# linum-uqam/ViT-OCM-WMSegmentation

Measured on AMD Instinct MI355X. Metric: OCM tiles/s (224x224, ViT-S/16 attention-map inference), higher is better.
Workload: dtype bf16x3

## Files before the change

include/ocm_vit.h:

```cpp
#ifndef OCM_VIT_H
#define OCM_VIT_H

#include <stddef.h>
#include <stdint.h>

#ifdef __cplusplus
extern "C" {
#endif

#define OCM_ABI_VERSION 16

enum {
    OCM_OK = 0,
    OCM_EINVAL = 1,
    OCM_ESTATE = 2,
    OCM_EHIP = 3,
    OCM_ENOMEM = 4,
    OCM_ENAME = 5
};

enum {
    OCM_PREC_BF16 = 0,
    OCM_PREC_FP32 = 1,
    OCM_PREC_BF16X3 = 2
// ... 82 lines not shown

int ocm_op_cast_bf16(const float *src, void *dst_bf16, size_t count, void *stream);
int ocm_op_cast_split(const float *src, void *dst_split, size_t count, void *stream);
int ocm_op_merge_split(const void *src_split, float *dst, size_t count, void *stream);

enum {
    OCM_EPI_BIAS_F32 = 0,
    OCM_EPI_BIAS_RESID_F32 = 1,
    OCM_EPI_BIAS_GELU_BF16 = 2,
    OCM_EPI_BIAS_BF16 = 3
};

int ocm_op_linear(int32_t precision, const void *a, const void *w, const float *bias, const float *resid,
                  void *out, int32_t M, int32_t N, int32_t K, int32_t epilogue, void *stream);

int ocm_linear_resid_ln_supported(int32_t D);
int ocm_op_linear_resid_ln(int32_t precision, const void *a, const void *w, const float *bias, const float *resid,
                           float *x, const float *gamma, const float *beta, void *xn, int32_t M, int32_t D, int32_t K,
                           float eps, void *stream);

int32_t ocm_n_pad(int32_t n_tokens);
int32_t ocm_n_pad_prec(int32_t precision, int32_t n_tokens);

int ocm_op_qkv_proj(int32_t precision, const void *a, const void *w, const float *bias, void *q, void *k,
                    void *vt, float *qkv_f32, int32_t batch, int32_t n_tokens, int32_t heads,
                    void *stream);

int ocm_op_attention(int32_t precision, const void *q, const void *k, const void *vt, void *ctx, float *lse2,
                     int32_t batch, int32_t n_tokens, int32_t heads, float scale, void *stream);

// ... 154 lines not shown
```

vit-ocm-wmsegmentation_amd/_lib.py:

```python
import ctypes as C
import os

_HERE = os.path.dirname(os.path.abspath(__file__))
LIB_PATH = os.environ.get("OCM_VIT_LIB") or os.path.join(_HERE, "libocm_vit.so")

OCM_ABI_VERSION = 16
OCM_OK, OCM_EINVAL, OCM_ESTATE, OCM_EHIP, OCM_ENOMEM, OCM_ENAME = 0, 1, 2, 3, 4, 5

OCM_PREC_BF16 = 0
OCM_PREC_FP32 = 1
OCM_PREC_BF16X3 = 2
OCM_SWIN_OPT_FUSE_MLP = 0
PRECISIONS = {"bf16": OCM_PREC_BF16, "fp32": OCM_PREC_FP32, "bf16x3": OCM_PREC_BF16X3}
DEFAULT_PRECISION = "bf16x3"
OCM_LN_F32, OCM_LN_BF16, OCM_LN_SPLIT = 0, 1, 2
OCM_OPT_FUSE_LN = 0
OCM_OPT_FOLD_LN = 1

OCM_OUT_FEAT = 1 << 0
OCM_OUT_ATTN = 1 << 1
OCM_OUT_QKV = 1 << 2
OCM_OUT_TOKENS = 1 << 3
OCM_OUT_ROWS = 1 << 4
OCM_LAST_ATTN_ONLY = 1 << 5
# ... 79 lines not shown
    "ocm_vit_destroy": (None, [_vp]),
    "ocm_vit_set_param": (C.c_int, [_vp, C.c_char_p, _vp, _sz, _vp]),
    "ocm_vit_params_ready": (C.c_int, [_vp]),
    "ocm_vit_workspace_bytes": (_sz, [_vp, _i32, _i32]),
    "ocm_vit_forward": (C.c_int, [_vp, C.POINTER(OcmVitIO)]),
    "ocm_vit_prepare_tokens": (C.c_int, [_vp, C.POINTER(OcmVitIO), _vp]),
    "ocm_vit_block_forward": (C.c_int, [_vp, _i32, _vp, _i32, _i32, _i32, _vp, _vp, _vp, _sz, _vp]),
    "ocm_vit_final_norm": (C.c_int, [_vp, _vp, _vp, _i64, _vp]),
    "ocm_op_layernorm": (C.c_int, [_vp, _vp, _vp, _vp, _i32, _i64, _i32, _f32, _vp]),
    "ocm_op_cast_bf16": (C.c_int, [_vp, _vp, _sz, _vp]),
    "ocm_op_cast_split": (C.c_int, [_vp, _vp, _sz, _vp]),
    "ocm_op_merge_split": (C.c_int, [_vp, _vp, _sz, _vp]),
    "ocm_n_pad_prec": (_i32, [_i32, _i32]),
    "ocm_op_linear": (C.c_int, [_i32, _vp, _vp, _vp, _vp, _vp, _i32, _i32, _i32, _i32, _vp]),
    "ocm_linear_resid_ln_supported": (C.c_int, [_i32]),
    "ocm_op_linear_resid_ln": (C.c_int, [_i32, _vp, _vp, _vp, _vp, _vp, _vp, _vp, _vp, _i32, _i32, _i32, _f32, _vp]),
    "ocm_n_pad": (_i32, [_i32]),
    "ocm_op_qkv_proj": (C.c_int, [_i32, _vp, _vp, _vp, _vp, _vp, _vp, _vp, _i32, _i32, _i32, _vp]),
    "ocm_op_attention": (C.c_int, [_i32, _vp, _vp, _vp, _vp, _vp, _i32, _i32, _i32, _f32, _vp]),
    "ocm_op_qkv_proj_hd": (C.c_int, [_i32, _vp, _vp, _vp, _vp, _vp, _vp, _vp, _i32, _i32, _i32, _i32, _vp]),
    "ocm_op_attention_hd": (C.c_int, [_i32, _vp, _vp, _vp, _vp, _vp, _i32, _i32, _i32, _i32, _f32, _vp]),
    "ocm_op_attention_probs_hd": (C.c_int, [_i32, _vp, _vp, _vp, _vp, _i32, _i32, _i32, _i32, _f32, _vp]),
    "ocm_op_attention_generic": (C.c_int, [C.c_int32, C.c_void_p, C.c_void_p, C.c_void_p, C.c_int32, C.c_int32, C.c_int32,
                                           C.c_int32, C.c_float, C.c_void_p]),
    "ocm_op_attention_probs": (C.c_int, [_i32, _vp, _vp, _vp, _vp, _i32, _i32, _i32, _f32, _vp]),
    "ocm_op_attention_rows": (C.c_int, [_i32, _vp, _vp, _vp, _i32, _vp, _i32, _i32, _i32, _f32, _vp]),
    "ocm_op_attention_map": (C.c_int, [_vp, _vp, _i32, _i32, _i32, _i32, _i32, _i32, _i32, _vp]),
    "ocm_op_tile_postprocess": (C.c_int, [_vp, _vp, _i32, _i32, _i32, _i32, _vp]),
    "ocm_op_bilinear_upsample": (C.c_int, [_vp, _vp, _i32, _i32, _i32, _i32, _vp]),
    "ocm_op_nearest_upsample": (C.c_int, [_vp, _vp, _i32, _i32, _i32, _i32, _vp]),
# ... 130 lines not shown
```

vit-ocm-wmsegmentation_amd/csrc/common.h:

```cpp
#pragma once
#include <hip/hip_runtime.h>
#include <stddef.h>
#include <stdint.h>

typedef __bf16 bf16;
typedef __bf16 bf16x2 __attribute__((ext_vector_type(2)));
typedef __bf16 bf16x4 __attribute__((ext_vector_type(4)));
typedef __bf16 bf16x8 __attribute__((ext_vector_type(8)));
typedef float f32x2 __attribute__((ext_vector_type(2)));
typedef float f32x4 __attribute__((ext_vector_type(4)));
typedef float f32x16 __attribute__((ext_vector_type(16)));

#define OCM_WAVE 64
#define OCM_HEAD_DIM 64

__device__ __forceinline__ int acc_row32(int reg, int h) { return (reg & 3) + 8 * (reg >> 2) + 4 * h; }

__device__ __forceinline__ int lds_off(int row, int chunk) {
    return row * 128 + ((chunk ^ ((row >> 1) & 7)) << 4);
}

__device__ __forceinline__ void lds_barrier() {
    __builtin_amdgcn_fence(__ATOMIC_RELEASE, "workgroup", "local");
    __builtin_amdgcn_s_barrier();
// ... 54 lines not shown
#if defined(OCM_ABL) && OCM_ABL == 1
    asm volatile("" ::"v"(ah), "v"(al), "v"(bh), "v"(bl));
    return c;
#endif
    c = __builtin_amdgcn_mfma_f32_32x32x16_bf16(al, bh, c, 0, 0, 0);
    c = __builtin_amdgcn_mfma_f32_32x32x16_bf16(ah, bl, c, 0, 0, 0);
    return __builtin_amdgcn_mfma_f32_32x32x16_bf16(ah, bh, c, 0, 0, 0);
}

typedef float f32x4_t __attribute__((ext_vector_type(4)));
__device__ __forceinline__ f32x4_t mfma16x3(bf16x8 ah, bf16x8 al, bf16x8 bh, bf16x8 bl, f32x4_t c) {
    c = __builtin_amdgcn_mfma_f32_16x16x32_bf16(al, bh, c, 0, 0, 0);
    c = __builtin_amdgcn_mfma_f32_16x16x32_bf16(ah, bl, c, 0, 0, 0);
    return __builtin_amdgcn_mfma_f32_16x16x32_bf16(ah, bh, c, 0, 0, 0);
}
__device__ __forceinline__ bf16x8 tr_read8(const char *p) {
#if defined(__HIP_DEVICE_COMPILE__)
    typedef short s16x4 __attribute__((ext_vector_type(4)));
    typedef __attribute__((address_space(3))) s16x4 *lds_s16x4;
    const s16x4 a = __builtin_amdgcn_ds_read_tr16_b64_v4i16((lds_s16x4)p);
    const s16x4 b = __builtin_amdgcn_ds_read_tr16_b64_v4i16((lds_s16x4)(p + 4 * 64));
    typedef short s16x8 __attribute__((ext_vector_type(8)));
    const s16x8 v = {a[0], a[1], a[2], a[3], b[0], b[1], b[2], b[3]};
    return __builtin_bit_cast(bf16x8, v);
#else
    return bf16x8{};
#endif
}

template <int ACCL>
__device__ __forceinline__ int acc_rpos(int e, int lane) {
    return ACCL ? 16 * (e >> 3) + 4 * ((lane >> 4) & 3) + (e & 3) : acc_row32(e, lane >> 5);
}
template <int ACCL>
__device__ __forceinline__ int acc_cpos(int e, int lane) {
    return ACCL ? 16 * ((e >> 2) & 1) + (lane & 15) : (lane & 31);
}

__device__ __forceinline__ int xcd_remap(int bid, int nwg) {
    const int q = nwg >> 3, r = nwg & 7, x = bid & 7;
    return (x < r ? x * (q + 1) : r * (q + 1) + (x - r) * q) + (bid >> 3);
}

__device__ __forceinline__ void xcd_remap2(int &bx, int &by) {
    const int id = xcd_remap(blockIdx.y * gridDim.x + blockIdx.x, gridDim.x * gridDim.y);
    by = id / (int)gridDim.x;
    bx = id - by * (int)gridDim.x;
}

__device__ __forceinline__ float fast_exp2(float x) { return __builtin_amdgcn_exp2f(x); }

// ... 37 lines not shown
```

vit-ocm-wmsegmentation_amd/csrc/engine.hip:

```cpp
#include <stdarg.h>
#include <stdio.h>
#include <string.h>

#include <atomic>
#include <mutex>
#include <string>
#include <vector>

#include "host_common.h"
#include "launch.h"
#include "dev_knobs.h"

static thread_local std::string g_err;

int ocm_fail(int code, const char *fmt, ...) {
    char buf[512];
    va_list ap;
    va_start(ap, fmt);
    vsnprintf(buf, sizeof buf, fmt, ap);
    va_end(ap);
    g_err = buf;
    return code;
}
#define fail ocm_fail
// ... 673 lines not shown
                             void *out, int32_t M, int32_t N, int32_t K, int32_t epilogue, void *stream) {
    int pc = 0, rc = prec_of(precision, &pc);
    if (rc) return rc;
    if (!a || !w || !out) return fail(OCM_EINVAL, "null argument");
    const int kq = pc ? 32 : 64;
    if (M <= 0 || N <= 0 || N % 32 || K <= 0 || K % kq)
        return fail(OCM_EINVAL, "bad shape M=%d N=%d K=%d (N%%32, K%%%d)", M, N, K, kq);
    if (pc == 2 && (epilogue == OCM_EPI_BIAS_GELU_BF16 || epilogue == OCM_EPI_BIAS_BF16) && N % 32)
        return fail(OCM_EINVAL, "split-pair outputs need N %% 32 == 0");
    if (epilogue < 0 || epilogue > 3) return fail(OCM_EINVAL, "bad epilogue %d", epilogue);
    if (epilogue == OCM_EPI_BIAS_RESID_F32 && !resid) return fail(OCM_EINVAL, "residual epilogue without resid");
    HIP_TRY(launch_linear(pc, a, w, bias, resid, out, M, N, K, epilogue, (hipStream_t)stream));
    return OCM_OK;
}

extern "C" int ocm_linear_resid_ln_supported(int32_t D) { return linear_resid_ln_supported(D) ? 1 : 0; }

extern "C" int ocm_op_linear_resid_ln(int32_t precision, const void *a, const void *w, const float *bias,
                                      const float *resid, float *x, const float *gamma, const float *beta, void *xn,
                                      int32_t M, int32_t D, int32_t K, float eps, void *stream) {
    int pc = 0, rc = prec_of(precision, &pc);
    if (rc) return rc;
    if (!a || !w || !resid || !x || !gamma || !beta || !xn) return fail(OCM_EINVAL, "null argument");
    if (!linear_resid_ln_supported(D)) return fail(OCM_EINVAL, "row width %d not in {128, 256, 384}", D);
    if (M <= 0 || K <= 0 || K % 64) return fail(OCM_EINVAL, "bad shape M=%d K=%d (K%%64)", M, K);
    HIP_TRY(launch_linear_resid_ln(pc, a, w, bias, resid, x, gamma, beta, xn, M, D, K, eps, (hipStream_t)stream));
    return OCM_OK;
}

static int op_qkv_proj(int32_t precision, const void *a, const void *w, const float *bias, void *q, void *k, void *vt,
// ... 303 lines not shown
```

vit-ocm-wmsegmentation_amd/csrc/gemm_core.h:

```cpp
#pragma once
#include <type_traits>
#include "common.h"

#ifdef OCM_GEMM_STAMPS
__device__ unsigned long long g_wstamps[512 * 16 * 8];
#define WSTAMP(k)                                                                                       \
    do {                                                                                                \
        if (t == nsteps / 2 && (threadIdx.x & 63) == 0 && blockIdx.x < 512)                              \
            g_wstamps[(blockIdx.x * 16 + (threadIdx.x >> 6 & 15)) * 8 + (k)] = __builtin_readcyclecounter(); \
    } while (0)
__device__ unsigned long long g_stamps[8192 * 8];
#define STAMP(i)                                                                                        \
    do {                                                                                                \
        if (threadIdx.x == 0 && blockIdx.x < 8192) g_stamps[blockIdx.x * 8 + (i)] = __builtin_readcyclecounter(); \
    } while (0)
#else
#define STAMP(i) ((void)0)
#define WSTAMP(k) ((void)0)
#endif

template <int BM_, int BN_, int WAVES_M_, int WAVES_N_, int MF16_ = 0>
struct GemmCfg {
    static constexpr int BM = BM_, BN = BN_, WAVES_M = WAVES_M_, WAVES_N = WAVES_N_, MF16 = MF16_;
    static constexpr int NT = WAVES_M * WAVES_N * OCM_WAVE;
// ... 53 lines not shown
#endif
        return *(const Raw *)(h + t * 128 + c * 16);
    }
    __device__ __forceinline__ static Raw finish(const Raw &r, int) { return r; }
};

template <class AL, class = void>
struct aload_w_tail {
    static constexpr bool v = false;
};
template <class AL>
struct aload_w_tail<AL, std::void_t<decltype(AL::W_TAIL)>> {
    static constexpr bool v = AL::W_TAIL;
};

template <class Cfg, class E, bool SWAP>
__device__ __forceinline__ void mma_step(const char *Ab, const char *Bb, int r, int h,
                                         f32x16 (&acc)[Cfg::TM][Cfg::TN], int wm = 0) {
    constexpr int TM = Cfg::TM, TN = Cfg::TN;
    static_assert(!Cfg::HALF || (Elem<E>::MODE == 2 && Cfg::MF16 && !SWAP), "half tiles exist on the 16 x 16 shape only");
    if constexpr (Elem<E>::MODE == 2 && Cfg::MF16) {
        const int r16 = r & 15, g = (r >> 4) + 2 * h;
        bf16x8 ah[TM][2], al[TM][2], bh[TN][2], bl[TN][2];
#pragma unroll
        for (int i = 0; i < TM; ++i)
#pragma unroll
            for (int ra = 0; ra < 2; ++ra) {
                if (Cfg::HALF && i == TM - 1) {
                    if (ra == 0) {
                        const char *Ah = Ab + ((TM - 1) * Cfg::RB - wm * 16) * 128;
                        ah[i][0] = *(const bf16x8 *)(Ah + lds_off(r16, g));
                        al[i][0] = *(const bf16x8 *)(Ah + lds_off(r16, 4 + g));
                    }
                    continue;
                }
                ah[i][ra] = *(const bf16x8 *)(Ab + i * Cfg::RB * 128 + lds_off(ra * 16 + r16, g));
                al[i][ra] = *(const bf16x8 *)(Ab + i * Cfg::RB * 128 + lds_off(ra * 16 + r16, 4 + g));
            }
#pragma unroll
        for (int j = 0; j < TN; ++j)
#pragma unroll
            for (int cb = 0; cb < 2; ++cb) {
                bh[j][cb] = *(const bf16x8 *)(Bb + j * Cfg::CB * 128 + lds_off(cb * 16 + r16, g));
                bl[j][cb] = *(const bf16x8 *)(Bb + j * Cfg::CB * 128 + lds_off(cb * 16 + r16, 4 + g));
            }
#pragma unroll
        for (int i = 0; i < TM; ++i)
#pragma unroll
            for (int j = 0; j < TN; ++j)
#pragma unroll
                for (int q = 0; q < ((Cfg::HALF && i == TM - 1) ? 2 : 4); ++q) {
                    f32x4_t c = __builtin_shufflevector(acc[i][j], acc[i][j], 0, 1, 2, 3);
                    if (q == 1) c = __builtin_shufflevector(acc[i][j], acc[i][j], 4, 5, 6, 7);
                    if (q == 2) c = __builtin_shufflevector(acc[i][j], acc[i][j], 8, 9, 10, 11);
                    if (q == 3) c = __builtin_shufflevector(acc[i][j], acc[i][j], 12, 13, 14, 15);
                    c = SWAP ? mfma16x3(bh[j][q >> 1], bl[j][q >> 1], ah[i][q & 1], al[i][q & 1], c)
                             : mfma16x3(ah[i][q >> 1], al[i][q >> 1], bh[j][q & 1], bl[j][q & 1], c);
#pragma unroll
                    for (int e = 0; e < 4; ++e) acc[i][j][4 * q + e] = c[e];
                }
    } else if constexpr (Elem<E>::MODE == 2) {
#pragma unroll
        for (int s = 0; s < 2; ++s) {
            bf16x8 ah[TM], al[TM], bh[TN], bl[TN];
#pragma unroll
            for (int i = 0; i < TM; ++i) {
                ah[i] = *(const bf16x8 *)(Ab + i * Cfg::RB * 128 + lds_off(r, 2 * s + h));
                al[i] = *(const bf16x8 *)(Ab + i * Cfg::RB * 128 + lds_off(r, 4 + 2 * s + h));
            }
#pragma unroll
            for (int j = 0; j < TN; ++j) {
// ... 234 lines not shown
        __builtin_amdgcn_raw_ptr_buffer_load_lds(rs, (lds_ptr)(img + (j * NW + wave) * 1024), 16, voff[j], soff, 0, AUX);
#endif
}

template <int CNT, int AUX = 0>
__device__ __forceinline__ void dma_pieces(__amdgpu_buffer_rsrc_t rs, char *img, const int (&voff)[CNT], const int (&piece)[CNT],
                                           int soff) {
#if defined(__HIP_DEVICE_COMPILE__)
    typedef __attribute__((address_space(3))) void *lds_ptr;
#pragma unroll
    for (int j = 0; j < CNT; ++j)
        __builtin_amdgcn_raw_ptr_buffer_load_lds(rs, (lds_ptr)(img + piece[j] * 1024), 16, voff[j], soff, 0, AUX);
#endif
}

template <class Cfg, class E, bool SWAP, int KSTEPS, int NSTAGE, int A_AUX = 0>
__device__ __forceinline__ void gemm_mainloop_dma(const E *__restrict__ A, int64_t lda, const E *__restrict__ W,
                                                  int64_t ldw, int m0, int n0, int M, int N, int K, char *smem,
                                                  f32x16 (&acc)[Cfg::TM][Cfg::TN], const float *__restrict__ bias) {
    constexpr int BM = Cfg::BM, BN = Cfg::BN, NT = Cfg::NT, NW = NT / 64;
    constexpr int TM = Cfg::TM, TN = Cfg::TN;
    constexpr int A_P = BM / 8, A_I = (A_P + NW - 1) / NW, B_I = BN / 8 / NW, LPS = A_I + B_I;
    constexpr int STAGE = (BM + BN) * 128, D = NSTAGE - 1;
    static_assert(BM % 8 == 0 && BN % (8 * NW) == 0 && (A_P % NW == 0 || 2 * (A_P % NW) >= NW), "each wave fills whole groups of 8 rows");
    static_assert(NSTAGE >= 2 && NSTAGE <= 4, "2..4 LDS stages");
    const int tid = threadIdx.x, lane = tid & 63;
    const int wave = __builtin_amdgcn_readfirstlane(tid >> 6);
    const int wm = wave / Cfg::WAVES_N, wn = wave % Cfg::WAVES_N;
    const int r = lane & 31, h = lane >> 5;
    const int esz = (int)sizeof(E);
    const int nsteps = KSTEPS > 0 ? KSTEPS : K / Elem<E>::KROW;

    auto bound = [](int64_t rows, int64_t ld_bytes) {
        const int64_t b = rows * ld_bytes;
// ... 4 lines not shown
    const auto rsB = __builtin_amdgcn_make_buffer_rsrc((void *)((const char *)W + (int64_t)n0 * ldw * esz), 0,
                                                       bound(N - n0, ldw * esz), 0x00020000);
    int voffA[A_I], voffB[B_I];
    int pieceA[A_I];
#pragma unroll
    for (int j = 0; j < A_I; ++j) {
        int pc = j * NW + wave;
        if (pc >= A_P) pc -= A_P % NW;
        pieceA[j] = pc;
        const int rho = pc * 8 + (lane >> 3);
        voffA[j] = rho * (int)(lda * esz) + (((lane & 7) ^ ((rho >> 1) & 7)) << 4);
    }
#pragma unroll
    for (int j = 0; j < B_I; ++j) {
        const int rho = (j * NW + wave) * 8 + (lane >> 3);
        voffB[j] = rho * (int)(ldw * esz) + (((lane & 7) ^ ((rho >> 1) & 7)) << 4);
    }
#define OCM_DMA_ISSUE(t, buf)                                                   \
    do {                                                                        \
        char *st_ = smem + (buf) * STAGE;                                       \
        dma_pieces<A_I, A_AUX>(rsA, st_, voffA, pieceA, (t) * 128);             \
        dma_rows<B_I, NW>(rsB, st_ + BM * 128, voffB, wave, (t) * 128);         \
    } while (0)
    auto compute = [&](int buf) {
        const char *st = smem + buf * STAGE;
        mma_step<Cfg, E, SWAP>(st + (wm * 32) * 128, st + BM * 128 + (wn * 32) * 128, r, h, acc, wm);
    };

    constexpr int ACCL = accl_of<Cfg, E>();
    constexpr int NBV = SWAP ? 16 : (ACCL ? 2 : 1);
    float bv[TN][NBV];
#pragma unroll
    for (int j = 0; j < TN; ++j) {
        const int nb = n0 + (j * Cfg::WAVES_N + wn) * 32;
#pragma unroll
        for (int e = 0; e < NBV; ++e)
            bv[j][e] = bias ? bias[min(nb + (SWAP ? acc_rpos<ACCL>(e, lane) : acc_cpos<ACCL>(4 * e, lane)), N - 1)] : 0.f;
    }
#pragma unroll
    for (int t = 0; t < D; ++t)
        if (t < nsteps) OCM_DMA_ISSUE(t, t);
#pragma unroll
    for (int j = 0; j < TN; ++j)
#pragma unroll
        for (int i = 0; i < TM; ++i)
#pragma unroll
            for (int e = 0; e < 16; ++e) acc[i][j][e] = bv[j][SWAP ? e : (ACCL ? ((e >> 2) & 1) : 0)];
    int bc = 0, bi = D % NSTAGE;
#ifdef OCM_GEMM_STAMPS
    unsigned long long stamp_wait = 0;
#endif
    for (int t = 0; t < nsteps; ++t) {
        const int younger = min(D - 1, nsteps - 1 - t);
#ifdef OCM_GEMM_STAMPS
        const unsigned long long tw0 = __builtin_readcyclecounter();
#endif
        WSTAMP(0);
        wait_vm_steps<LPS, NSTAGE - 2>(younger);
        WSTAMP(1);
#ifdef OCM_GEMM_STAMPS
        const unsigned long long tw1 = __builtin_readcyclecounter();
#endif
        raw_barrier();
#ifdef OCM_GEMM_STAMPS
        if (t == 0) STAMP(6);
        if (t > 0) {
            const unsigned long long tw2 = __builtin_readcyclecounter();
            stamp_wait += ((tw2 - tw1) << 32) | ((tw1 - tw0) & 0xFFFFFFFFull);
        }
#endif
        WSTAMP(2);
#if !defined(OCM_ABL) || OCM_ABL != 2
        if (t + D < nsteps) OCM_DMA_ISSUE(t + D, bi);
#endif
        __builtin_amdgcn_sched_barrier(0);
        WSTAMP(3);
        compute(bc);
#ifdef OCM_GEMM_STAMPS
        if (t == nsteps / 2) {
            __builtin_amdgcn_sched_barrier(0);
            asm volatile("v_mov_b32 %0, %0\n\ts_nop 0" : "+v"(acc[TM - 1][TN - 1][15]));
            WSTAMP(4);
        }
#endif
        bc = bc + 1 == NSTAGE ? 0 : bc + 1;
        bi = bi + 1 == NSTAGE ? 0 : bi + 1;
    }
    raw_barrier();
#ifdef OCM_GEMM_STAMPS
    if (threadIdx.x == 0 && blockIdx.x < 8192) g_stamps[blockIdx.x * 8 + 7] = stamp_wait;
#endif
#undef OCM_DMA_ISSUE
}

constexpr int EPI_MAXS = 6;
struct EpiPre {
    f32x2 raw[EPI_MAXS];
    f32x2 cd;
};
struct EpiNoPre {};
template <class Cfg, class Epi>
__device__ __forceinline__ auto epi_prefetch(const Epi &epi, int m0, int n0, int M, int N) {
    if constexpr (Epi::ROWTAB) {
// ... 71 lines not shown
        constexpr int NBUF = 2 * PASS <= LDS_AVAIL ? 2 : 1;
#pragma unroll
        for (int j = 0; j < Cfg::TN; ++j) {
            if (NBUF == 1 && j) lds_barrier();
            float *C = (float *)(smem + (j % NBUF) * PASS);
            if (active)
#pragma unroll
            for (int i = 0; i < Cfg::TM; ++i) {
                const int col0 = (i * Cfg::WAVES_M + wm) * 32;
#pragma unroll
                for (int e = 0; e < 16; ++e)
                    C[(wn * 32 + acc_rpos<ACCL>(e, lane)) * Cfg::BM + col0 + acc_cpos<ACCL>(e, lane)] = acc[i][j][e];
            }
            lds_barrier();
            if (active) epi.template run<PassCfg<Cfg::BM, Cfg::CB, Cfg::NT>>((const float *)C, m0, n0 + j * Cfg::CB, rowtab, coltab + j * Cfg::CB);
        }
    }
}

template <class Cfg, class E, bool SWAP, int KSTEPS, int NSTAGE, class Epi, int A_AUX = 0>
__global__ __launch_bounds__(Cfg::NT) void gemm_dma_kernel(const E *__restrict__ A, int64_t lda, const E *__restrict__ W,
                                                           int64_t ldw, int M, int N, int K, Epi epi) {
    extern __shared__ __attribute__((aligned(16))) char smem[];
    const int tiles_n = (N + Cfg::BN - 1) / Cfg::BN;
    const int id = xcd_remap(blockIdx.x, gridDim.x);
    const int tm = id / tiles_n, tn = id - tm * tiles_n;
    const int m0 = tm * Cfg::BM, n0 = tn * Cfg::BN;
    f32x16 acc[Cfg::TM][Cfg::TN];
    const auto pre = epi_prefetch<Cfg>(epi, m0, n0, M, N);
    STAMP(0);
#if defined(OCM_ABL) && OCM_ABL == 4
#pragma unroll
    for (int i = 0; i < Cfg::TM; ++i)
#pragma unroll
        for (int j = 0; j < Cfg::TN; ++j)
#pragma unroll
            for (int e = 0; e < 16; ++e) acc[i][j][e] = (float)(threadIdx.x + e);
#else
    gemm_mainloop_dma<Cfg, E, SWAP, KSTEPS, NSTAGE, A_AUX>(A, lda, W, ldw, m0, n0, M, N, K, smem, acc, epi.bias);
#endif
    STAMP(1);
#if defined(OCM_ABL) && OCM_ABL == 3
#pragma unroll
    for (int i = 0; i < Cfg::TM; ++i)
#pragma unroll
        for (int j = 0; j < Cfg::TN; ++j) asm volatile("" ::"v"(acc[i][j]));
#else
    run_epilogue<Cfg, SWAP, Epi, NSTAGE * (Cfg::BM + Cfg::BN) * 128, decltype(pre), accl_of<Cfg, E>()>(acc, smem, epi, m0, n0, true, &pre);
#endif
    STAMP(4);
#ifdef OCM_GEMM_STAMPS
    __builtin_amdgcn_s_waitcnt(0);
    STAMP(5);
// ... 24 lines not shown
```

vit-ocm-wmsegmentation_amd/csrc/gemm_kernels.h:

```cpp
#pragma once
#include <type_traits>
#include "gemm_core.h"
#include "launch.h"
#include "dev_knobs.h"

int ocm_wt_mask();

#ifndef OCM_SMALLM_STAGES
#define OCM_SMALLM_STAGES 4
#endif
constexpr int OCM_SMALLM_ROWS = 4096;
typedef GemmCfg<128, 128, 2, 2> Cfg128x128;
typedef GemmCfg<128, 128, 2, 4> Cfg128x128q;
typedef GemmCfg<128, 128, 2, 4, 1> Cfg128x128q16;
typedef GemmCfg<128, 128, 2, 2, 1> Cfg128x128m16;
typedef GemmCfg<160, 128, 2, 4, 1> Cfg160x128q16;
typedef GemmCfg<256, 256, 2, 4, 1> Cfg256x256m16;
typedef GemmCfg<64, 128, 2, 2> Cfg64x128;
typedef GemmCfg<64, 128, 2, 4> Cfg64x128w;
typedef GemmCfg<64, 64, 2, 2> Cfg64x64;
typedef GemmCfg<256, 256, 2, 4> Cfg256x256;

static inline bool big_tiles_pay(int M, int N, int K) {
    return K >= 768 && N % 256 == 0 && (long)((M + 255) / 256) * (N / 256) >= 512;
// ... 61 lines not shown
}
__device__ __forceinline__ f32x2 ln_col_entry(const LnFold &ln, int n) {
    return ln.stats ? f32x2{ln.c[n], ln.d[n]} : f32x2{0.f, 0.f};
}

template <int MODE, class OE>
struct EpiLinear {
    const float *bias;
    const float *resid;
    void *out;
    int M, N;
    int64_t ldo;
    int wt = 0;
    LnFold ln;
    static constexpr bool ROWTAB = (MODE == 2 || MODE == 3);
    __device__ __forceinline__ void row_raw(int m, f32x2 (&raw)[EPI_MAXS]) const { ln_row_raw(ln, m, raw); }
    __device__ __forceinline__ f32x2 row_final(const f32x2 (&raw)[EPI_MAXS]) const { return ln_row_final(ln, raw); }
    __device__ __forceinline__ f32x2 col_entry(int n) const { return ln_col_entry(ln, n); }
    template <class Cfg>
    __device__ __forceinline__ void run(const float *C, int m0, int n0, const f32x2 *rowtab, const f32x2 *coltab) const {
        constexpr int BM = Cfg::BM, BN = Cfg::BN, NT = Cfg::NT;
        constexpr bool ACT_OUT = (MODE == 2 || MODE == 3);
        constexpr int W = ACT_OUT ? Elem<OE>::EPW : 4;
        constexpr int CPR = BN / W;
        constexpr int TOTAL = BM * CPR, ITERS = (TOTAL + NT - 1) / NT;
        f32x4 rs[MODE == 1 ? ITERS : 1];
        if (MODE == 1) {
#pragma unroll
            for (int i = 0; i < ITERS; ++i) {
                const int q = min((int)threadIdx.x + i * NT, TOTAL - 1), row = q / CPR, col = (q - row * CPR) * W;
// ... 21 lines not shown
                    const f32x2 mr = rowtab[row];
                    const float mu = mr[0], rstd = mr[1];
#pragma unroll
                    for (int e = 0; e < 4; ++e) {
                        const f32x2 cd = coltab[col + e];
                        v0[e] = fmaf(rstd, fmaf(-mu, cd[0], v0[e]), cd[1]);
                    }
                    if (W == 8) {
#pragma unroll
                        for (int e = 0; e < 4; ++e) {
                            const f32x2 cd = coltab[col + 4 + e];
                            v1[e] = fmaf(rstd, fmaf(-mu, cd[0], v1[e]), cd[1]);
                        }
                    }
                }
                if (MODE == 2) {
#pragma unroll
                    for (int e = 0; e < 4; e += 2) {
                        const f32x2 a = gelu_erf2(f32x2{v0[e], v0[e + 1]});
                        v0[e] = a[0];
                        v0[e + 1] = a[1];
                        if (W == 8) {
                            const f32x2 b = gelu_erf2(f32x2{v1[e], v1[e + 1]});
                            v1[e] = b[0];
                            v1[e + 1] = b[1];
                        }
                    }
                }
                if (wt)
                    store_act_wt((OE *)nullptr, (char *)out + (int64_t)m * ldo * (int)sizeof(OE), n, v0, v1);
                else
                    store_act((OE *)nullptr, (char *)out + (int64_t)m * ldo * (int)sizeof(OE), n, v0, v1);
            }
        }
    }
};

template <class OE>
struct EpiResidStats {
    static constexpr bool ROWTAB = false;
    static constexpr int BN_MULT = 64;
    const float *bias;
    const float *resid;
    float *x;
    void *xs;
    float *stats;
    int M, N;
// ... 157 lines not shown
typedef GemmCfg<128, 192, 4, 2> Cfg128x192;
typedef GemmCfg<128, 256, 2, 4> Cfg128x256;
typedef GemmCfg<128, 96, 4, 1> Cfg128x96;
template <class Epi, class = void>
struct epi_bn_mult {
    static constexpr int v = 1;
};
template <class Epi>
struct epi_bn_mult<Epi, std::void_t<decltype(Epi::BN_MULT)>> {
    static constexpr int v = Epi::BN_MULT;
};

template <int MODE, class E, class Epi>
static hipError_t launch_linear_epi(const E *a, const E *w, const Epi &epi, int M, int N, int K, hipStream_t s) {
    RowLoader<E> al{a, K};
    if constexpr (Elem<E>::MODE == 2) {
#ifdef OCM_DEV
        switch (OCM_KNOB(0)) {
            case -1: goto reg_staged;
            case 1: if (N % 256 == 0) return launch_gemm_dma<Cfg256x256, E, 2>(a, K, w, K, M, N, K, epi, s); break;
            case 4: if (N % 128 == 0) return launch_gemm_dma<Cfg128x128, E, 2>(a, K, w, K, M, N, K, epi, s); break;
            case 6: if (N % 128 == 0) return launch_gemm_dma<Cfg256x128, E, 2>(a, K, w, K, M, N, K, epi, s); break;
            case 7: if (N % 128 == 0) return launch_gemm_dma<Cfg64x128, E, 2>(a, K, w, K, M, N, K, epi, s); break;
            case 8: if (N % 128 == 0) return launch_gemm_dma<Cfg64x128, E, 3>(a, K, w, K, M, N, K, epi, s); break;
            case 9: if (N % 128 == 0) return launch_gemm_dma<Cfg64x128, E, 4>(a, K, w, K, M, N, K, epi, s); break;
            case 10: if (N % 64 == 0) return launch_gemm_dma<Cfg64x64, E, 4>(a, K, w, K, M, N, K, epi, s); break;
            case 11: if (N == 384) return launch_gemm_dma<Cfg128x192, E, 3>(a, K, w, K, M, N, K, epi, s); break;
            case 12: if (N % 128 == 0) return launch_gemm_dma<Cfg128x128q, E, 2>(a, K, w, K, M, N, K, epi, s); break;
            case 13: if (N % 128 == 0) return launch_gemm_dma<Cfg128x128q16, E, 2>(a, K, w, K, M, N, K, epi, s); break;
            case 14: if (N % 128 == 0) return launch_gemm_dma<Cfg128x128m16, E, 2>(a, K, w, K, M, N, K, epi, s); break;
// ... 716 lines not shown
```

vit-ocm-wmsegmentation_amd/csrc/kernels_gemm.hip:

```cpp
#include "launch.h"
#include "dev_knobs.h"

template <class E>
hipError_t launch_linear_e(const E *a, const E *w, const float *bias, const float *resid, void *out, int M, int N, int K,
                           int epilogue, hipStream_t s, const LnFold &ln, const StatsOut &so);
template <class E>
hipError_t launch_linear_ld_e(const E *a, int64_t lda, const E *w, const float *bias, const float *resid, void *out,
                              int64_t ldo, int M, int N, int K, int epilogue, hipStream_t s);
template <class E>
hipError_t launch_resid_ln_e(const E *a, const E *w, const float *bias, const float *resid, float *x, const float *gamma,
                             const float *beta, void *xn, int M, int D, int K, float eps, hipStream_t s);
template <class E>
hipError_t launch_qkv_e(const E *a, const E *w, const float *bias, E *q, E *k, E *vt, float *qkv_f32, int batch,
                        int n_tokens, int n_pad, int heads, int head_dim, bool want_v, hipStream_t s, const LnFold &ln);
template <class E>
hipError_t launch_patch_e(const PatchArgs &pa, const E *w, const float *bias, const float *pos, float *x, int dim,
                          hipStream_t s, const StatsOut &so);

#ifdef OCM_DEV
int g_ocm_knobs[8] = {0, 0, 0, 0, 0, 0, 0, 0};
#endif
int ocm_wt_mask() { return OCM_KNOB(1) == 0 ? 35 : OCM_KNOB(1) < 0 ? 0 : OCM_KNOB(1); }

hipError_t launch_linear_ld(int prec, const void *a, int64_t lda, const void *w, const float *bias, const float *resid,
                            void *out, int64_t ldo, int M, int N, int K, int epilogue, hipStream_t s) {
    if (prec == 2) return hipErrorInvalidValue;
    if (prec)
        return launch_linear_ld_e<float>((const float *)a, lda, (const float *)w, bias, resid, out, ldo, M, N, K, epilogue,
                                         s);
    return launch_linear_ld_e<bf16>((const bf16 *)a, lda, (const bf16 *)w, bias, resid, out, ldo, M, N, K, epilogue, s);
}

hipError_t launch_linear(int prec, const void *a, const void *w, const float *bias, const float *resid, void *out, int M,
                         int N, int K, int epilogue, hipStream_t s, const LnFold &ln, const StatsOut &so) {
    if (prec == 2) return launch_linear_e<sp32>((const sp32 *)a, (const sp32 *)w, bias, resid, out, M, N, K, epilogue, s, ln, so);
    if (prec) return launch_linear_e<float>((const float *)a, (const float *)w, bias, resid, out, M, N, K, epilogue, s, ln, so);
    return launch_linear_e<bf16>((const bf16 *)a, (const bf16 *)w, bias, resid, out, M, N, K, epilogue, s, ln, so);
// ... 35 lines not shown
```

vit-ocm-wmsegmentation_amd/csrc/launch.h:

```cpp
#pragma once
#include <atomic>
#include "common.h"

typedef std::atomic<unsigned long long> OptinMask;
static inline hipError_t lds_optin(const void *kern, int bytes, OptinMask &done) {
    int dev = 0;
    if (hipError_t e = hipGetDevice(&dev); e != hipSuccess) return e;
    const unsigned long long bit = 1ull << (dev & 63);
    if (done.load(std::memory_order_acquire) & bit) return hipSuccess;
    const hipError_t e = hipFuncSetAttribute(kern, hipFuncAttributeMaxDynamicSharedMemorySize, bytes);
    if (e == hipSuccess) done.fetch_or(bit, std::memory_order_release);
    return e;
}

hipError_t launch_layernorm(const float *x, const float *gamma, const float *beta, void *y, int out_kind,
                            int64_t rows, int dim, float eps, hipStream_t s);
static inline int ln_kind_of_prec(int prec) { return prec == 0 ? 1 : prec == 1 ? 0 : 2; }
hipError_t launch_cast_bf16(const float *src, bf16 *dst, size_t count, hipStream_t s);
hipError_t launch_cast_split(const float *src, void *dst, size_t count, hipStream_t s);
hipError_t launch_merge_split(const void *src, float *dst, size_t count, hipStream_t s);
hipError_t launch_fold_split(const float *src, void *dst, int D, int C, int pp, hipStream_t s);
hipError_t launch_fold_cast_bf16(const float *src, bf16 *dst, int D, int C, int pp, hipStream_t s);
hipError_t launch_fold_f32(const float *src, float *dst, int D, int C, int pp, hipStream_t s);
hipError_t launch_im2col3x3(int prec, const float *in, void *out, int batch, int h, int w, int C, int relu, hipStream_t s);
// ... 15 lines not shown
    const float *tok_shift = nullptr;
    float *part = nullptr;
};
constexpr int OCM_SPLITK = 4, OCM_SPLITK_MAX_ROWS = 512;
hipError_t launch_splitk_finish(const float *part, int slices, const float *bias, const float *resid, float *x, void *xs,
                                float *stats, int M, int N, hipStream_t s, const StatsOut &so = StatsOut());
hipError_t launch_cls_rows_stats(const float *cls, const float *pos, float *x, void *xs, float *stats, int batch,
                                 int n_tokens, int dim, hipStream_t s, float *shift = nullptr, float *tok_shift = nullptr,
                                 const float *pe_bias = nullptr);
hipError_t launch_fold_ln(const float *W, const float *gamma, const float *beta, const float *bias, void *Wf, float *cvec,
                          float *dvec, int N, int K, hipStream_t s);

hipError_t launch_linear(int prec, const void *a, const void *w, const float *bias, const float *resid, void *out, int M,
                         int N, int K, int epilogue, hipStream_t s, const LnFold &ln = LnFold(),
                         const StatsOut &so = StatsOut());
bool linear_resid_ln_supported(int D);
hipError_t launch_linear_resid_ln(int prec, const void *a, const void *w, const float *bias, const float *resid, float *x,
                                  const float *gamma, const float *beta, void *xn, int M, int D, int K, float eps,
                                  hipStream_t s);
hipError_t launch_qkv(int prec, const void *a, const void *w, const float *bias, void *q, void *k, void *vt,
                      float *qkv_f32, int batch, int n_tokens, int n_pad, int heads, int head_dim, bool want_v,
                      hipStream_t s, const LnFold &ln = LnFold());
hipError_t launch_attention_generic(int prec, const float *qkv, void *ctx, float *attn, const int32_t *query_rows,
                                    int n_rows, float *rows, int batch, int n_tokens, int heads, int head_dim, float scale,
                                    hipStream_t s);
struct PatchArgs {
    const float *image;
    int64_t sb, sc, sy;
    const int32_t *origins;
    int batch, hp, wp, p, chans;
// ... 80 lines not shown
```

Baseline: 28970.

## Store bf16 GEMM epilogue directly from registers using a transposed MFMA order

For split-bf16 GEMMs with bias or bias+GELU bf16 epilogues on 128-wide N tiles, the mainloop now runs in swapped operand order with a permuted W row mapping. Each lane then holds eight contiguous output columns, so the epilogue stores straight from accumulators instead of staging the tile through LDS. The LN-fold row and column tables are published to LDS just before the last k-step, and the final barrier is dropped. A forced-tile test entry point is also added. This risks bank conflicts or correctness issues from the new row permutation.

```diff
diff --git a/include/ocm_vit.h b/include/ocm_vit.h
--- a/include/ocm_vit.h
+++ b/include/ocm_vit.h
@@ -120,6 +120,9 @@
 int ocm_op_linear(int32_t precision, const void *a, const void *w, const float *bias, const float *resid,
                   void *out, int32_t M, int32_t N, int32_t K, int32_t epilogue, void *stream);
 
+int ocm_op_linear_tile(int32_t precision, const void *a, const void *w, const float *bias, void *out, int32_t M, int32_t N,
+                       int32_t K, int32_t epilogue, int32_t tile_rows, void *stream);
+
 int ocm_linear_resid_ln_supported(int32_t D);
 int ocm_op_linear_resid_ln(int32_t precision, const void *a, const void *w, const float *bias, const float *resid,
                            float *x, const float *gamma, const float *beta, void *xn, int32_t M, int32_t D, int32_t K,
diff --git a/vit-ocm-wmsegmentation_amd/_lib.py b/vit-ocm-wmsegmentation_amd/_lib.py
--- a/vit-ocm-wmsegmentation_amd/_lib.py
+++ b/vit-ocm-wmsegmentation_amd/_lib.py
@@ -117,6 +117,7 @@
     "ocm_n_pad_prec": (_i32, [_i32, _i32]),
     "ocm_op_linear": (C.c_int, [_i32, _vp, _vp, _vp, _vp, _vp, _i32, _i32, _i32, _i32, _vp]),
     "ocm_linear_resid_ln_supported": (C.c_int, [_i32]),
+    "ocm_op_linear_tile": (C.c_int, [_i32, _vp, _vp, _vp, _vp, _i32, _i32, _i32, _i32, _i32, _vp]),
     "ocm_op_linear_resid_ln": (C.c_int, [_i32, _vp, _vp, _vp, _vp, _vp, _vp, _vp, _vp, _i32, _i32, _i32, _f32, _vp]),
     "ocm_n_pad": (_i32, [_i32]),
     "ocm_op_qkv_proj": (C.c_int, [_i32, _vp, _vp, _vp, _vp, _vp, _vp, _vp, _i32, _i32, _i32, _vp]),
diff --git a/vit-ocm-wmsegmentation_amd/csrc/common.h b/vit-ocm-wmsegmentation_amd/csrc/common.h
--- a/vit-ocm-wmsegmentation_amd/csrc/common.h
+++ b/vit-ocm-wmsegmentation_amd/csrc/common.h
@@ -92,6 +92,11 @@
     c = __builtin_amdgcn_mfma_f32_16x16x32_bf16(ah, bl, c, 0, 0, 0);
     return __builtin_amdgcn_mfma_f32_16x16x32_bf16(ah, bh, c, 0, 0, 0);
 }
+__device__ __forceinline__ f32x4_t mfma16x3_t(bf16x8 ah, bf16x8 al, bf16x8 bh, bf16x8 bl, f32x4_t c) {
+    c = __builtin_amdgcn_mfma_f32_16x16x32_bf16(bh, al, c, 0, 0, 0);
+    c = __builtin_amdgcn_mfma_f32_16x16x32_bf16(bl, ah, c, 0, 0, 0);
+    return __builtin_amdgcn_mfma_f32_16x16x32_bf16(bh, ah, c, 0, 0, 0);
+}
 __device__ __forceinline__ bf16x8 tr_read8(const char *p) {
 #if defined(__HIP_DEVICE_COMPILE__)
     typedef short s16x4 __attribute__((ext_vector_type(4)));
@@ -113,6 +118,12 @@
 template <int ACCL>
 __device__ __forceinline__ int acc_cpos(int e, int lane) {
     return ACCL ? 16 * ((e >> 2) & 1) + (lane & 15) : (lane & 31);
+}
+
+__device__ __forceinline__ int acc_t_npos(int e, int lane) { return 8 * ((lane >> 4) & 3) + 4 * (e >> 3) + (e & 3); }
+__device__ __forceinline__ int acc_t_mpos(int e, int lane) { return 16 * ((e >> 2) & 1) + (lane & 15); }
+__device__ __forceinline__ int acc_t_wrow(int rho) {
+    return (rho & ~31) | (((rho >> 2) & 3) << 3) | (((rho >> 4) & 1) << 2) | (rho & 3);
 }
 
 __device__ __forceinline__ int xcd_remap(int bid, int nwg) {
diff --git a/vit-ocm-wmsegmentation_amd/csrc/engine.hip b/vit-ocm-wmsegmentation_amd/csrc/engine.hip
--- a/vit-ocm-wmsegmentation_amd/csrc/engine.hip
+++ b/vit-ocm-wmsegmentation_amd/csrc/engine.hip
@@ -711,6 +711,23 @@
     return OCM_OK;
 }
 
+struct ForcedTile {
+    explicit ForcedTile(int rows) { ocm_set_forced_tile(rows); }
+    ~ForcedTile() { ocm_set_forced_tile(0); }
+};
+
+extern "C" int ocm_op_linear_tile(int32_t precision, const void *a, const void *w, const float *bias, void *out, int32_t M,
+                                  int32_t N, int32_t K, int32_t epilogue, int32_t tile_rows, void *stream) {
+    if (precision != OCM_PREC_BF16X3) return fail(OCM_EINVAL, "named tiles exist in split-bf16 precision");
+    if (!a || !w || !out) return fail(OCM_EINVAL, "null argument");
+    if (tile_rows != 128 && tile_rows != 160) return fail(OCM_EINVAL, "tile_rows %d not in {128, 160}", tile_rows);
+    if (epilogue != OCM_EPI_BIAS_GELU_BF16 && epilogue != OCM_EPI_BIAS_BF16) return fail(OCM_EINVAL, "bad epilogue %d", epilogue);
+    if (M <= 0 || N <= 0 || N % 128 || K <= 0 || K % 32) return fail(OCM_EINVAL, "bad shape M=%d N=%d K=%d (N%%128, K%%32)", M, N, K);
+    ForcedTile ft(tile_rows);
+    HIP_TRY(launch_linear(2, a, w, bias, nullptr, out, M, N, K, epilogue, (hipStream_t)stream));
+    return OCM_OK;
+}
+
 extern "C" int ocm_linear_resid_ln_supported(int32_t D) { return linear_resid_ln_supported(D) ? 1 : 0; }
 
 extern "C" int ocm_op_linear_resid_ln(int32_t precision, const void *a, const void *w, const float *bias,
diff --git a/vit-ocm-wmsegmentation_amd/csrc/gemm_core.h b/vit-ocm-wmsegmentation_amd/csrc/gemm_core.h
--- a/vit-ocm-wmsegmentation_amd/csrc/gemm_core.h
+++ b/vit-ocm-wmsegmentation_amd/csrc/gemm_core.h
@@ -91,11 +91,11 @@
     static constexpr bool v = AL::W_TAIL;
 };
 
-template <class Cfg, class E, bool SWAP>
+template <class Cfg, class E, bool SWAP, bool TORD = false>
 __device__ __forceinline__ void mma_step(const char *Ab, const char *Bb, int r, int h,
                                          f32x16 (&acc)[Cfg::TM][Cfg::TN], int wm = 0) {
     constexpr int TM = Cfg::TM, TN = Cfg::TN;
-    static_assert(!Cfg::HALF || (Elem<E>::MODE == 2 && Cfg::MF16 && !SWAP), "half tiles exist on the 16 x 16 shape only");
+    static_assert(!Cfg::HALF || (Elem<E>::MODE == 2 && Cfg::MF16 && (!SWAP || TORD)), "half tiles exist on the 16 x 16 shape only");
     if constexpr (Elem<E>::MODE == 2 && Cfg::MF16) {
         const int r16 = r & 15, g = (r >> 4) + 2 * h;
         bf16x8 ah[TM][2], al[TM][2], bh[TN][2], bl[TN][2];
@@ -126,12 +126,14 @@
 #pragma unroll
             for (int j = 0; j < TN; ++j)
 #pragma unroll
-                for (int q = 0; q < ((Cfg::HALF && i == TM - 1) ? 2 : 4); ++q) {
+                for (int q = 0; q < 4; ++q) {
+                    if (Cfg::HALF && i == TM - 1 && (SWAP ? (q & 1) : (q >> 1))) continue;
                     f32x4_t c = __builtin_shufflevector(acc[i][j], acc[i][j], 0, 1, 2, 3);
                     if (q == 1) c = __builtin_shufflevector(acc[i][j], acc[i][j], 4, 5, 6, 7);
                     if (q == 2) c = __builtin_shufflevector(acc[i][j], acc[i][j], 8, 9, 10, 11);
                     if (q == 3) c = __builtin_shufflevector(acc[i][j], acc[i][j], 12, 13, 14, 15);
-                    c = SWAP ? mfma16x3(bh[j][q >> 1], bl[j][q >> 1], ah[i][q & 1], al[i][q & 1], c)
+                    c = SWAP ? (TORD ? mfma16x3_t(ah[i][q & 1], al[i][q & 1], bh[j][q >> 1], bl[j][q >> 1], c)
+                                     : mfma16x3(bh[j][q >> 1], bl[j][q >> 1], ah[i][q & 1], al[i][q & 1], c))
                              : mfma16x3(ah[i][q >> 1], al[i][q >> 1], bh[j][q & 1], bl[j][q & 1], c);
 #pragma unroll
                     for (int e = 0; e < 4; ++e) acc[i][j][4 * q + e] = c[e];
@@ -396,10 +398,15 @@
 #endif
 }
 
-template <class Cfg, class E, bool SWAP, int KSTEPS, int NSTAGE, int A_AUX = 0>
+struct NoLastHook {
+    __device__ __forceinline__ void operator()() const {}
+};
+template <class Cfg, class E, bool SWAP, int KSTEPS, int NSTAGE, int A_AUX = 0, bool DIRECT = false, class Last = NoLastHook>
 __device__ __forceinline__ void gemm_mainloop_dma(const E *__restrict__ A, int64_t lda, const E *__restrict__ W,
                                                   int64_t ldw, int m0, int n0, int M, int N, int K, char *smem,
-                                                  f32x16 (&acc)[Cfg::TM][Cfg::TN], const float *__restrict__ bias) {
+                                                  f32x16 (&acc)[Cfg::TM][Cfg::TN], const float *__restrict__ bias,
+                                                  const Last &last = Last()) {
+    static_assert(!DIRECT || (SWAP && Elem<E>::MODE == 2 && Cfg::MF16), "the direct epilogue's accumulator layout");
     constexpr int BM = Cfg::BM, BN = Cfg::BN, NT = Cfg::NT, NW = NT / 64;
     constexpr int TM = Cfg::TM, TN = Cfg::TN;
     constexpr int A_P = BM / 8, A_I = (A_P + NW - 1) / NW, B_I = BN / 8 / NW, LPS = A_I + B_I;
@@ -434,7 +441,7 @@
 #pragma unroll
     for (int j = 0; j < B_I; ++j) {
         const int rho = (j * NW + wave) * 8 + (lane >> 3);
-        voffB[j] = rho * (int)(ldw * esz) + (((lane & 7) ^ ((rho >> 1) & 7)) << 4);
+        voffB[j] = (DIRECT ? acc_t_wrow(rho) : rho) * (int)(ldw * esz) + (((lane & 7) ^ ((rho >> 1) & 7)) << 4);
     }
 #define OCM_DMA_ISSUE(t, buf)                                                   \
     do {                                                                        \
@@ -444,7 +451,7 @@
     } while (0)
     auto compute = [&](int buf) {
         const char *st = smem + buf * STAGE;
-        mma_step<Cfg, E, SWAP>(st + (wm * 32) * 128, st + BM * 128 + (wn * 32) * 128, r, h, acc, wm);
+        mma_step<Cfg, E, SWAP, DIRECT>(st + (wm * 32) * 128, st + BM * 128 + (wn * 32) * 128, r, h, acc, wm);
     };
 
     constexpr int ACCL = accl_of<Cfg, E>();
@@ -455,7 +462,7 @@
         const int nb = n0 + (j * Cfg::WAVES_N + wn) * 32;
 #pragma unroll
         for (int e = 0; e < NBV; ++e)
-            bv[j][e] = bias ? bias[min(nb + (SWAP ? acc_rpos<ACCL>(e, lane) : acc_cpos<ACCL>(4 * e, lane)), N - 1)] : 0.f;
+            bv[j][e] = bias ? bias[min(nb + (DIRECT ? acc_t_npos(e, lane) : SWAP ? acc_rpos<ACCL>(e, lane) : acc_cpos<ACCL>(4 * e, lane)), N - 1)] : 0.f;
     }
 #pragma unroll
     for (int t = 0; t < D; ++t)
@@ -481,6 +488,7 @@
 #ifdef OCM_GEMM_STAMPS
         const unsigned long long tw1 = __builtin_readcyclecounter();
 #endif
+        if (DIRECT && t == nsteps - 1) last();
         raw_barrier();
 #ifdef OCM_GEMM_STAMPS
         if (t == 0) STAMP(6);
@@ -506,7 +514,7 @@
         bc = bc + 1 == NSTAGE ? 0 : bc + 1;
         bi = bi + 1 == NSTAGE ? 0 : bi + 1;
     }
-    raw_barrier();
+    if constexpr (!DIRECT) raw_barrier();
 #ifdef OCM_GEMM_STAMPS
     if (threadIdx.x == 0 && blockIdx.x < 8192) g_stamps[blockIdx.x * 8 + 7] = stamp_wait;
 #endif
@@ -608,6 +616,71 @@
             }
             lds_barrier();
             if (active) epi.template run<PassCfg<Cfg::BM, Cfg::CB, Cfg::NT>>((const float *)C, m0, n0 + j * Cfg::CB, rowtab, coltab + j * Cfg::CB);
+        }
+    }
+}
+
+template <class Epi, class = void>
+struct epi_has_store8 {
+    static constexpr bool v = false;
+};
+template <class Epi>
+struct epi_has_store8<Epi, std::void_t<decltype(Epi::STORE8)>> {
+    static constexpr bool v = Epi::STORE8;
+};
+template <class Cfg, class E, class Epi>
+constexpr bool epi_direct_ok() {
+    return Elem<E>::MODE == 2 && Cfg::MF16 && Cfg::BN == 128 && Cfg::WAVES_M == 2 && Cfg::WAVES_N == 4 && epi_has_store8<Epi>::v;
+}
+
+template <class Cfg, int LDS_AVAIL, class Epi, class Pre>
+__device__ __forceinline__ void epi_publish(char *smem, const Epi &epi, const Pre &pre) {
+    if constexpr (Epi::ROWTAB) {
+        f32x2 *rowtab = (f32x2 *)(smem + LDS_AVAIL), *coltab = rowtab + Cfg::BM;
+        if (threadIdx.x < Cfg::BM) rowtab[threadIdx.x] = epi.row_final(pre.raw);
+        if (threadIdx.x < Cfg::BN) coltab[threadIdx.x] = pre.cd;
+    }
+}
+
+template <class Cfg, int LDS_AVAIL, class Epi>
+__device__ __forceinline__ void run_epilogue_direct(const f32x16 (&acc)[Cfg::TM][Cfg::TN], const char *smem, const Epi &epi,
+                                                    int m0, int n0) {
+    const f32x2 *rowtab = (const f32x2 *)(smem + LDS_AVAIL), *coltab = rowtab + Cfg::BM;
+    const int lane = threadIdx.x & 63, wave = threadIdx.x >> 6;
+    const int wm = wave / Cfg::WAVES_N, wn = wave % Cfg::WAVES_N;
+    bool fold = false;
+    if constexpr (Epi::ROWTAB) fold = epi.ln.stats != nullptr;
+#pragma unroll
+    for (int j = 0; j < Cfg::TN; ++j) {
+        const int col = (j * Cfg::WAVES_N + wn) * 32 + acc_t_npos(0, lane);
+        if (n0 + col >= epi.ncols()) continue;
+        f32x2 cd[8];
+#pragma unroll
+        for (int e = 0; e < 8; ++e) cd[e] = fold ? coltab[col + e] : f32x2{0.f, 0.f};
+#pragma unroll
+        for (int i = 0; i < Cfg::TM; ++i) {
+            const bool half = Cfg::HALF && i == Cfg::TM - 1;
+            const int tm = half ? (Cfg::TM - 1) * Cfg::RB + wm * 16 : (i * Cfg::WAVES_M + wm) * 32;
+#pragma unroll
+            for (int mh = 0; mh < (half ? 1 : 2); ++mh) {
+                const int row = tm + acc_t_mpos(4 * mh, lane), m = m0 + row;
+                if (m >= epi.M) continue;
+                f32x4 v0, v1;
+#pragma unroll
+                for (int e = 0; e < 4; ++e) {
+                    v0[e] = acc[i][j][4 * mh + e];
+                    v1[e] = acc[i][j][8 + 4 * mh + e];
+                }
+                if (fold) {
+                    const f32x2 mr = rowtab[row];
+#pragma unroll
+                    for (int e = 0; e < 4; ++e) {
+                        v0[e] = fmaf(mr[1], fmaf(-mr[0], cd[e][0], v0[e]), cd[e][1]);
+                        v1[e] = fmaf(mr[1], fmaf(-mr[0], cd[4 + e][0], v1[e]), cd[4 + e][1]);
+                    }
+                }
+                epi.store8(m, n0 + col, v0, v1);
+            }
         }
     }
 }
@@ -631,6 +704,19 @@
 #pragma unroll
             for (int e = 0; e < 16; ++e) acc[i][j][e] = (float)(threadIdx.x + e);
 #else
+    constexpr int RING = NSTAGE * (Cfg::BM + Cfg::BN) * 128;
+    if constexpr (!SWAP && epi_direct_ok<Cfg, E, Epi>()) {
+        gemm_mainloop_dma<Cfg, E, true, KSTEPS, NSTAGE, A_AUX, true>(A, lda, W, ldw, m0, n0, M, N, K, smem, acc, epi.bias,
+                                                                     [&]() { epi_publish<Cfg, RING>(smem, epi, pre); });
+        STAMP(1);
+        run_epilogue_direct<Cfg, RING>(acc, smem, epi, m0, n0);
+        STAMP(4);
+#ifdef OCM_GEMM_STAMPS
+        __builtin_amdgcn_s_waitcnt(0);
+        STAMP(5);
+#endif
+        return;
+    }
     gemm_mainloop_dma<Cfg, E, SWAP, KSTEPS, NSTAGE, A_AUX>(A, lda, W, ldw, m0, n0, M, N, K, smem, acc, epi.bias);
 #endif
     STAMP(1);
diff --git a/vit-ocm-wmsegmentation_amd/csrc/gemm_kernels.h b/vit-ocm-wmsegmentation_amd/csrc/gemm_kernels.h
--- a/vit-ocm-wmsegmentation_amd/csrc/gemm_kernels.h
+++ b/vit-ocm-wmsegmentation_amd/csrc/gemm_kernels.h
@@ -5,6 +5,7 @@
 #include "dev_knobs.h"
 
 int ocm_wt_mask();
+int ocm_forced_tile();
 
 #ifndef OCM_SMALLM_STAGES
 #define OCM_SMALLM_STAGES 4
@@ -99,6 +100,27 @@
     int wt = 0;
     LnFold ln;
     static constexpr bool ROWTAB = (MODE == 2 || MODE == 3);
+    static constexpr bool STORE8 = (MODE == 2 || MODE == 3) && Elem<OE>::MODE == 2;
+    __device__ __forceinline__ int ncols() const { return N; }
+    __device__ __forceinline__ void store8(int m, int n, f32x4 v0, f32x4 v1) const {
+        if (MODE == 2) {
+#pragma unroll
+            for (int e = 0; e < 4; e += 2) {
+                const f32x2 a = gelu_erf2(f32x2{v0[e], v0[e + 1]});
+                v0[e] = a[0];
+                v0[e + 1] = a[1];
+                if (Elem<OE>::EPW == 8) {
+                    const f32x2 b = gelu_erf2(f32x2{v1[e], v1[e + 1]});
+                    v1[e] = b[0];
+                    v1[e + 1] = b[1];
+                }
+            }
+        }
+        if (wt)
+            store_act_wt((OE *)nullptr, (char *)out + (int64_t)m * ldo * (int)sizeof(OE), n, v0, v1);
+        else
+            store_act((OE *)nullptr, (char *)out + (int64_t)m * ldo * (int)sizeof(OE), n, v0, v1);
+    }
     __device__ __forceinline__ void row_raw(int m, f32x2 (&raw)[EPI_MAXS]) const { ln_row_raw(ln, m, raw); }
     __device__ __forceinline__ f32x2 row_final(const f32x2 (&raw)[EPI_MAXS]) const { return ln_row_final(ln, raw); }
     __device__ __forceinline__ f32x2 col_entry(int n) const { return ln_col_entry(ln, n); }
@@ -150,23 +172,7 @@
                         }
                     }
                 }
-                if (MODE == 2) {
-#pragma unroll
-                    for (int e = 0; e < 4; e += 2) {
-                        const f32x2 a = gelu_erf2(f32x2{v0[e], v0[e + 1]});
-                        v0[e] = a[0];
-                        v0[e + 1] = a[1];
-                        if (W == 8) {
-                            const f32x2 b = gelu_erf2(f32x2{v1[e], v1[e + 1]});
-                            v1[e] = b[0];
-                            v1[e + 1] = b[1];
-                        }
-                    }
-                }
-                if (wt)
-                    store_act_wt((OE *)nullptr, (char *)out + (int64_t)m * ldo * (int)sizeof(OE), n, v0, v1);
-                else
-                    store_act((OE *)nullptr, (char *)out + (int64_t)m * ldo * (int)sizeof(OE), n, v0, v1);
+                store8(m, n, v0, v1);
             }
         }
     }
@@ -354,6 +360,14 @@
 template <int MODE, class E, class Epi>
 static hipError_t launch_linear_epi(const E *a, const E *w, const Epi &epi, int M, int N, int K, hipStream_t s) {
     RowLoader<E> al{a, K};
+    if constexpr (Elem<E>::MODE == 2 && (MODE == 2 || MODE == 3)) {
+        if (const int ft = ocm_forced_tile(); ft) {
+            if (N % 128) return hipErrorInvalidValue;
+            if (ft == 128) return launch_gemm_dma<Cfg128x128q16, E, 2>(a, K, w, K, M, N, K, epi, s);
+            if (ft == 160) return launch_gemm_dma<Cfg160x128q16, E, 2>(a, K, w, K, M, N, K, epi, s);
+            return hipErrorInvalidValue;
+        }
+    }
     if constexpr (Elem<E>::MODE == 2) {
 #ifdef OCM_DEV
         switch (OCM_KNOB(0)) {
diff --git a/vit-ocm-wmsegmentation_amd/csrc/kernels_gemm.hip b/vit-ocm-wmsegmentation_amd/csrc/kernels_gemm.hip
--- a/vit-ocm-wmsegmentation_amd/csrc/kernels_gemm.hip
+++ b/vit-ocm-wmsegmentation_amd/csrc/kernels_gemm.hip
@@ -21,6 +21,10 @@
 int g_ocm_knobs[8] = {0, 0, 0, 0, 0, 0, 0, 0};
 #endif
 int ocm_wt_mask() { return OCM_KNOB(1) == 0 ? 35 : OCM_KNOB(1) < 0 ? 0 : OCM_KNOB(1); }
+
+static thread_local int t_forced_tile = 0;
+int ocm_forced_tile() { return t_forced_tile; }
+void ocm_set_forced_tile(int rows) { t_forced_tile = rows; }
 
 hipError_t launch_linear_ld(int prec, const void *a, int64_t lda, const void *w, const float *bias, const float *resid,
                             void *out, int64_t ldo, int M, int N, int K, int epilogue, hipStream_t s) {
diff --git a/vit-ocm-wmsegmentation_amd/csrc/launch.h b/vit-ocm-wmsegmentation_amd/csrc/launch.h
--- a/vit-ocm-wmsegmentation_amd/csrc/launch.h
+++ b/vit-ocm-wmsegmentation_amd/csrc/launch.h
@@ -53,6 +53,7 @@
 hipError_t launch_linear(int prec, const void *a, const void *w, const float *bias, const float *resid, void *out, int M,
                          int N, int K, int epilogue, hipStream_t s, const LnFold &ln = LnFold(),
                          const StatsOut &so = StatsOut());
+void ocm_set_forced_tile(int rows);
 bool linear_resid_ln_supported(int D);
 hipError_t launch_linear_resid_ln(int prec, const void *a, const void *w, const float *bias, const float *resid, float *x,
                                   const float *gamma, const float *beta, void *xn, int M, int D, int K, float eps,
```

After: 28910, median of 2. About the same (-0.2%).
